# ArsamAryandoust/CarParkingMaps

Measured on AMD Instinct MI355X. Metric: car-steps/sec at Z=4,096, 1k cars/zone; 1/2/4/8 MI355X + %HBM roofline, higher is better.
Workload: dtype f64

## Files before the change

### carparkingmaps_amd/csrc/cpm_grouped.h

```cpp
#pragma once
#include <hip/hip_runtime.h>
#include <stdint.h>

#include <algorithm>
#include <cstring>
#include <type_traits>
#include <string>

#include "../../include/cpm.h"
#include "cpm_kernels.h"
#include "cpm_dispatch.h"
#include "cpm_narrow.h"
#include "cpm_flows.h"
#include "cpm_flows_csr.h"
#include "cpm_stays.h"
#include "cpm_paths.h"
#include "cpm_charge.h"

namespace cpm {

constexpr int kFusedThreads = 256;
constexpr int kMaxZonesPerGroup = 1024;
constexpr uint32_t kHiMax = 0xFFFFFFFFu;
constexpr int kMaxCapMult = 64;
// ... 153 lines not shown
    int Z, Zq, G;
    int hour;
    uint32_t *done_t;
    int lag;
    uint32_t heavy_x;
    uint32_t spin_limit;
    const uint32_t *pD, *pcntg;
    int pchunks;
    uint32_t cap, scap, idbits, gdiv, step;
    CarIndex cars;
    uint64_t seed;
    int Zc;
    int smap;
    uint32_t *sdone;
    const uint32_t *psdone;
    uint32_t *pdone;
    uint32_t chained;
    const uint32_t *perm_t;
};


__device__ __forceinline__ void lds_barrier() { asm volatile("s_waitcnt lgkmcnt(0)\n\ts_barrier" ::: "memory"); }

__device__ __forceinline__ unsigned long long ballot64(bool p) { return __builtin_amdgcn_ballot_w64(p); }
__device__ __forceinline__ uint32_t xcc_id() { return __builtin_amdgcn_s_getreg((20) | (0 << 6) | (3 << 11)) & 15u; }
__device__ __forceinline__ uint32_t wave_incl_scan(uint32_t x)
{
    int v = static_cast<int>(x);
    v += __builtin_amdgcn_update_dpp(0, v, 0x111, 0xf, 0xf, false);
    v += __builtin_amdgcn_update_dpp(0, v, 0x112, 0xf, 0xf, false);
    v += __builtin_amdgcn_update_dpp(0, v, 0x114, 0xf, 0xf, false);
    v += __builtin_amdgcn_update_dpp(0, v, 0x118, 0xf, 0xf, false);
    v += __builtin_amdgcn_update_dpp(0, v, 0x142, 0xa, 0xf, false);
    v += __builtin_amdgcn_update_dpp(0, v, 0x143, 0xc, 0xf, false);
    return static_cast<uint32_t>(v);
}
__device__ __forceinline__ bool any64(bool p) { return __builtin_amdgcn_ballot_w64(p) != 0ull; }
template <int POLICY, typename W>
__device__ __forceinline__ void next_store(W v, W *p);
template <int POLICY = 0>
__device__ __forceinline__ void put32(uint32_t *p, uint32_t i, uint32_t v)
{
    next_store<POLICY>(v, reinterpret_cast<uint32_t *>(reinterpret_cast<char *>(p) + (i << 2)));
}
__device__ __forceinline__ uint32_t from_lane0(uint32_t v) { return static_cast<uint32_t>(__builtin_amdgcn_readfirstlane(static_cast<int>(v))); }

constexpr int kRowTile = 64;
constexpr int kRowBlock = 256;
constexpr int kCkptStride = 32;
__host__ __device__ inline int ckpt_count(int Z) { return (Z + kCkptStride - 1) / kCkptStride; }
constexpr size_t kRowLds = sizeof(double) * 2 * kRowTile * (kRowTile + 1) + sizeof(uint32_t) * kRowTile;

typedef uint32_t cpm_u32x2 __attribute__((ext_vector_type(2)));
typedef uint32_t cpm_u32x4 __attribute__((ext_vector_type(4)));
__device__ __forceinline__ double row_load(__amdgpu_buffer_rsrc_t rows, uint32_t lane_off, uint32_t row_off)
{
    const cpm_u32x2 v = __builtin_amdgcn_raw_buffer_load_b64(rows, lane_off, row_off, 0);
    return __hiloint2double(static_cast<int>(v.y), static_cast<int>(v.x));
}

__device__ __forceinline__ void row_sums(double (*tile)[kRowTile][kRowTile + 1], const double *__restrict__ src, int lane, bool live,
                                         double *__restrict__ ck, double *__restrict__ last_o, int Z, int nt, int *err)
{
    constexpr int H = kRowTile / 2;
    const uint32_t lane_off = static_cast<uint32_t>(live ? lane : 0) << 3;
    const size_t Zs = static_cast<size_t>(Z);
    const uint32_t rowb = static_cast<uint32_t>(Z) * 8u;
    double run = 0.0;
    bool bad = false;
    double xa[H], xb[H];
    auto window = [&](const double *row0) {
        return __builtin_amdgcn_make_buffer_rsrc(const_cast<double *>(row0), 0, static_cast<int>(2 * kRowTile * rowb), 0x00020000);
    };
    auto sums = [&](double(&x)[H], int buf, int jbase, double *ck_slot) {
#pragma unroll
        for (int u = 0; u < H; ++u) {
            bad |= !(x[u] >= 0.0);
            run = run + x[u];
            tile[buf][lane][jbase + u] = run;
        }
        if (ck_slot && live) *ck_slot = run;
    };
    const int nfull = Z / kRowTile;
    const double *row0 = src;
    __amdgpu_buffer_rsrc_t rows = window(row0);
    if (nfull > 0) {
#pragma unroll
        for (int u = 0; u < H; ++u) xa[u] = row_load(rows, lane_off, static_cast<uint32_t>(u) * rowb);
    }
#pragma unroll 1
    for (int k = 0; k + 1 < nfull; ++k) {
#pragma unroll
        for (int u = 0; u < H; ++u) xb[u] = row_load(rows, lane_off, static_cast<uint32_t>(H + u) * rowb);
        sums(xa, k & 1, 0, ck ? ck + static_cast<size_t>(2 * k) * Zs : nullptr);
#pragma unroll
        for (int u = 0; u < H; ++u) xa[u] = row_load(rows, lane_off, static_cast<uint32_t>(kRowTile + u) * rowb);
        sums(xb, k & 1, H, ck ? ck + static_cast<size_t>(2 * k + 1) * Zs : nullptr);
        lds_barrier();
        row0 += kRowTile * Zs;
        rows = window(row0);
    }
    if (nfull > 0) {
        const int k = nfull - 1;
#pragma unroll
        for (int u = 0; u < H; ++u) xb[u] = row_load(rows, lane_off, static_cast<uint32_t>(H + u) * rowb);
        sums(xa, k & 1, 0, ck ? ck + static_cast<size_t>(2 * k) * Zs : nullptr);
// ... 456 lines not shown
__host__ __device__ constexpr int policy_sorted(int p) { return (p >> 2) & 3; }
__host__ __device__ constexpr int policy_medium(int p) { return (p >> 4) & 3; }
__host__ __device__ constexpr int policy_surplus(int p) { return (p >> 6) & 3; }
__host__ __device__ constexpr int policy_pack_aux(int p) { return ((p >> 8) & 1) ? 2 : 0; }
#ifndef CPM_HOUR_STAY
#define CPM_HOUR_STAY 0
#endif
#ifndef CPM_HOUR_SORTED
#define CPM_HOUR_SORTED 0
#endif
#ifndef CPM_HOUR_MEDIUM
#define CPM_HOUR_MEDIUM 0
#endif
#ifndef CPM_HOUR_SURPLUS
#define CPM_HOUR_SURPLUS 0
#endif
#ifndef CPM_HOUR_PACK_NT
#define CPM_HOUR_PACK_NT 1
#endif
#ifndef CPM_PAIR_STAY
#define CPM_PAIR_STAY 0
#endif
#ifndef CPM_PAIR_SORTED
#define CPM_PAIR_SORTED 0
#endif
#ifndef CPM_PAIR_SURPLUS
#define CPM_PAIR_SURPLUS 0
#endif
#ifndef CPM_PAIR_PACK_NT
#define CPM_PAIR_PACK_NT 1
#endif
#ifndef CPM_ZERO_STORE
#define CPM_ZERO_STORE 0
#endif
__host__ __device__ constexpr int policy_dense_pack_only(int p, bool sparse) { return sparse ? (p & 0xFF) : p; }
constexpr int kPolicyHour = store_policy(CPM_HOUR_STAY, CPM_HOUR_SORTED, CPM_HOUR_MEDIUM, CPM_HOUR_SURPLUS, CPM_HOUR_PACK_NT);
constexpr int kPolicyPair = store_policy(CPM_PAIR_STAY, CPM_PAIR_SORTED, 0, CPM_PAIR_SURPLUS, CPM_PAIR_PACK_NT);
template <bool FUSED>
__device__ __forceinline__ uint32_t hand_load(const uint32_t *p)
{
    if constexpr (FUSED) return __hip_atomic_load(p, __ATOMIC_RELAXED, __HIP_MEMORY_SCOPE_AGENT);
    else return *p;
}
template <bool FUSED>
__device__ __forceinline__ void hand_off_done(uint32_t *done_chunk, int tid)
{
    if constexpr (FUSED) {
        asm volatile("s_waitcnt vmcnt(0)" ::: "memory");
        __builtin_amdgcn_s_barrier();
        if (tid == 0) __hip_atomic_fetch_add(done_chunk, 1u, __ATOMIC_RELAXED, __HIP_MEMORY_SCOPE_AGENT);
    }
}

template <int BLOCK, int CPT, int NQ, bool GROUPED, bool FUSED, bool WAIT = false, bool SPARSE = false, bool STAGED = false, int POLICY = 0, bool NARROW = false>
__device__ __forceinline__ void grouped_sample_body(const GroupedArgs &a, const int z, uint32_t *pack, SampleLds &sl, uint32_t *done_chunk,
                                                    const uint32_t *wait_on = nullptr, uint32_t wait_need = 0)
{
    static_assert(!(STAGED && (WAIT || FUSED)), "a staged pack is the batched sampler's: two launches per hour");
    static_assert(!NARROW || (FUSED && GROUPED && !WAIT && !SPARSE && !STAGED), "narrow packs: the one-launch hour on dense tables");
    uint32_t &s_ndrive = sl.ndrive, &s_nstay = sl.nstay, &s_split = sl.split;
    uint32_t(&gb)[kGroups] = sl.gb;
    uint32_t(&stage)[kGroups * kStage] = sl.stage;
    const int tid = threadIdx.x, lane = tid & 63;
    const uint32_t cap = a.cap;
    const uint32_t b = static_cast<uint32_t>(z) * cap;
    const int gw = pack_guide_words(a.G), rw = NARROW ? narrow_row_words(a.Zq, a.G) : pack_row_words(a.Zq, a.G, SPARSE ? 1 : 0), pieces = rw / 4, sh = 32 - a.G;
    CPM_SSTAMP_DECL;
    CPM_SSTAMP(0);
    uint32_t ns_raw = a.cnt_s[z];
    if constexpr (WAIT) ns_raw &= kCntMask;
    const double last = a.last_t[z];
    const long long thr = a.thr_t[z];
    uint32_t na_raw;
    uint32_t id[CPT + 1];
    if constexpr (WAIT) {
        typedef uint32_t u32x2 __attribute__((ext_vector_type(2)));
        u32x2 seen = {wait_need, 0u};
        const bool poller = wait_need && tid < 64;
        if (poller) asm volatile("global_load_dwordx2 %0, %1, %2 sc1" : "=v"(seen) : "v"(0), "s"(wait_on) : "memory");
        pack_dma<BLOCK, NQ>(pack, a.rp_t + static_cast<size_t>(z) * rw, pieces, tid);
        if (poller) {
            asm volatile("s_waitcnt vmcnt(%1)" : "+v"(seen) : "n"(NQ) : "memory");
            uint32_t got = from_lane0(seen.x), where = from_lane0(seen.y);
            for (uint32_t spins = 0; (got & kDoneCount) < wait_need; ++spins) {
                if (spins >= a.spin_limit) break;
                __builtin_amdgcn_s_sleep(32);
                got = from_lane0(lane == 0 ? __hip_atomic_load(wait_on, __ATOMIC_RELAXED, __HIP_MEMORY_SCOPE_AGENT) : 0u);
                where = from_lane0(lane == 0 ? __hip_atomic_load(wait_on + 1, __ATOMIC_RELAXED, __HIP_MEMORY_SCOPE_AGENT) : 0u);
            }
            const bool bad = (got & kDoneCount) < wait_need || (got >> 16) != 0u || where != (1u << xcc_id());
            if (bad && lane == 0) atomicOr(a.rare->status, 4ull);
            if (tid == 0) sl.pad_ = bad ? 1u : 0u;
        }
        bool dead = false;
        if (wait_need) {
            lds_barrier();
            dead = sl.pad_ != 0u;
        }
        const uint32_t nsc = dead ? 0u : min(ns_raw, cap);
        uint32_t nav = 0;
        if (!dead) {
            asm volatile("global_load_dword %0, %1, %2 sc1" : "=v"(nav) : "v"(0), "s"(a.cnt_a + z) : "memory");
#pragma unroll
            for (int c = 0; c <= CPT; ++c) {
                const uint32_t s1 = static_cast<uint32_t>(tid + c * BLOCK);
                const uint32_t pos = s1 < nsc ? s1 : (cap - 1u + nsc - min(s1, cap - 1u + nsc));
                asm volatile("global_load_dword %0, %1, %2 sc1" : "=v"(id[c]) : "v"(pos << 2), "s"(a.ids + b) : "memory");
// ... 24 lines not shown
            asm volatile("global_load_dword %0, %1, %2" : "=v"(id[c]) : "v"(off), "s"(a.ids + b) : "memory");
        }
        if constexpr (STAGED) {
            wait_ids<CPT + 1, 0>(id);
        } else {
            pack_dma<BLOCK, NQ, policy_pack_aux(POLICY)>(pack, a.rp_t + static_cast<size_t>(z) * rw, pieces, tid);
            wait_ids<CPT + 1, NQ>(id);
        }
    }
    CPM_SSTAMP(1);
    const bool heavy = n_all > a.heavy_x * (CPT > 4 ? 4 : CPT) * BLOCK;
    if (tid == 0) {
        a.parking_t[z] = n_all;
        if (static_cast<unsigned long long>(ns_raw) + na_raw > cap) atomicOr(a.rare->status, 2ull);
        s_ndrive = 0;
        s_nstay = 0;
        uint32_t split = 0;
        if (heavy) {
            const GroupedRare *r = a.rare;
            const uint32_t items = (n_all + CPT * BLOCK - 1) / (CPT * BLOCK) - 1u;
            atomicMax(&r->maxn[0], n_all);
            const uint32_t idx = atomicAdd(r->nheavy + a.hour, items);
            atomicMax(&r->maxn[1], idx + items);
            if (GROUPED && r->parts > 1) {
                if (idx + items <= r->hgrid) {
                    for (uint32_t q = 0; q < items; ++q) r->heavy_list[idx + q] = static_cast<uint32_t>(z) | (q << 16);
                    split = 1;
                } else {
                    for (uint32_t q = 0; q < items && idx + q < r->hgrid; ++q) r->heavy_list[idx + q] = 0xFFFFFFFFu;
                }
            }
        }
        s_split = split;
    }
    if (tid < kGroups) gb[tid] = 0;
    if (n_all == 0) {
        if (GROUPED) {
            if (tid == 0) a.cnt_next[z] = 0;
            if (tid < kGroups) hand_store<FUSED>(&a.cntg[static_cast<size_t>(z) * kGroups + tid], 0u);
        }
        asm volatile("s_waitcnt vmcnt(0)" ::: "memory");
        hand_off_done<FUSED>(done_chunk, tid);
        return;
    }
    uint32_t nd = 0;
    uint32_t n = 0;
    const unsigned long long below = (1ull << lane) - 1ull;
    uint32_t *stay_out = a.ids_next + static_cast<size_t>(z) * cap;
    uint32_t *runs = GROUPED ? a.D + static_cast<size_t>(z) * kGroups * a.scap : nullptr;
    const uint16_t *guide = reinterpret_cast<const uint16_t *>(pack);
    const uint32_t *hi = pack + gw;
    const uint16_t *smap = SPARSE ? reinterpret_cast<const uint16_t *>(hi + a.Zq) : nullptr;
    uint32_t hi_last = 0;
    auto first_pass = [&](auto kc) {
        constexpr int K = decltype(kc)::value;
        bool valid[K ? K : 1], drive[K ? K : 1], want[K ? K : 1], ok[K ? K : 1];
        uint32_t dest[K ? K : 1], clo[K ? K : 1], khi[K ? K : 1];
#pragma unroll
        for (int c = 0; c < K; ++c) {
            valid[c] = static_cast<uint32_t>(tid + c * BLOCK) < n_all;
            long long kb;
            car_draw_words(a.seed, a.cars.global(id[c]), a.step, kb, clo[c], khi[c]);
            drive[c] = valid[c] & (kb <= thr);
            want[c] = drive[c] & (last != 0.0);
        }
        CPM_SSTAMP(2);
        asm volatile("s_waitcnt vmcnt(0)" ::: "memory");
        __syncthreads();
        CPM_SSTAMP(3);
        n = s_split ? static_cast<uint32_t>(CPT * BLOCK) : n_all;
        if constexpr (NARROW) hi_last = hi[0];
        else hi_last = hi[(SPARSE ? a.Zc : a.Z) - 1];
        if constexpr (K > 0) {
            if constexpr (NARROW) narrow_pack_search<K>(pack, gw, khi, want, sh, hi_last, a.Z, a.Zq, a.rare, a.hour, z, dest, ok);
            else pack_search<K>(guide, hi, khi, want, sh, hi_last, a.Zq, dest, ok, smap);
            {
                bool anyx = false;
#pragma unroll
                for (int c = 0; c < K; ++c) {
                    dest[c] = want[c] ? dest[c] : static_cast<uint32_t>(z);
                    anyx |= want[c] & !ok[c];
                }
                if (__builtin_expect(any64(anyx), 0)) {
#pragma unroll
                    for (int c = 0; c < K; ++c) {
                        if (want[c] & !ok[c]) {
                            if constexpr (NARROW) {
                                long long kb;
                                car_draw_words(a.seed, a.cars.global(id[c]), a.step, kb, clo[c], khi[c]);
                            }
                            dest[c] = search_exact_any<SPARSE>(a.rare, a.hour, z, u53(clo[c], khi[c]), last, khi[c] <= hi_last ? static_cast<int>(dest[c]) : -1);
                        }
                    }
                }
            }
            CPM_SSTAMP(4);
            if (GROUPED) {
                unsigned long long mS[K];
                uint32_t total = 0;
#pragma unroll
                for (int c = 0; c < K; ++c) {
                    mS[c] = ballot64(valid[c] & !drive[c]);
                    total += static_cast<uint32_t>(__popcll(mS[c]));
                }
                uint32_t bS = 0;
                if (lane == 0 && total) bS = atomicAdd(&s_nstay, total);
                bS = from_lane0(bS);
                uint32_t rank[K];
#pragma unroll
                for (int c = 0; c < K; ++c) rank[c] = drive[c] ? atomicAdd(&gb[gdiv_group_t<SPARSE>(a.gdiv, dest[c])], 1u) : 0u;
#pragma unroll
                for (int c = 0; c < K; ++c) {
                    if (valid[c] & !drive[c]) put32<policy_stay(POLICY)>(stay_out, bS + static_cast<uint32_t>(__popcll(mS[c] & below)), id[c]);
                    bS += static_cast<uint32_t>(__popcll(mS[c]));
                }
#pragma unroll
                for (int c = 0; c < K; ++c) {
                    if (drive[c]) {
                        const uint32_t g = gdiv_group_t<SPARSE>(a.gdiv, dest[c]);
                        const uint32_t packed = id[c] | (gdiv_local_t<SPARSE>(a.gdiv, dest[c], g) << a.idbits);
                        if (rank[c] < static_cast<uint32_t>(kStage)) stage[g * kStage + rank[c]] = packed;
                        else if (rank[c] < a.scap) hand_store<FUSED>(&runs[g * a.scap + rank[c]], packed);
                    }
                }
            } else {
#pragma unroll
// ... 16 lines not shown
            case 4: first_pass(std::integral_constant<int, 4>{}); break;
            case 5: first_pass(std::integral_constant<int, 5>{}); break;
            case 6: first_pass(std::integral_constant<int, 6>{}); break;
            case 7: first_pass(std::integral_constant<int, 7>{}); break;
            default: first_pass(std::integral_constant<int, 8>{}); break;
            }
        } else if constexpr (CPT == 7) {
            switch (k) {
            case 0: first_pass(std::integral_constant<int, 0>{}); break;
            case 1: first_pass(std::integral_constant<int, 1>{}); break;
            case 2: first_pass(std::integral_constant<int, 2>{}); break;
            case 3: first_pass(std::integral_constant<int, 3>{}); break;
            case 4: first_pass(std::integral_constant<int, 4>{}); break;
            case 5: first_pass(std::integral_constant<int, 5>{}); break;
            case 6: first_pass(std::integral_constant<int, 6>{}); break;
            default: first_pass(std::integral_constant<int, 7>{}); break;
            }
        } else if constexpr (CPT == 6) {
            switch (k) {
            case 0: first_pass(std::integral_constant<int, 0>{}); break;
            case 1: first_pass(std::integral_constant<int, 1>{}); break;
            case 2: first_pass(std::integral_constant<int, 2>{}); break;
            case 3: first_pass(std::integral_constant<int, 3>{}); break;
            case 4: first_pass(std::integral_constant<int, 4>{}); break;
            case 5: first_pass(std::integral_constant<int, 5>{}); break;
            default: first_pass(std::integral_constant<int, 6>{}); break;
            }
        } else if constexpr (CPT == 5) {
            switch (k) {
            case 0: first_pass(std::integral_constant<int, 0>{}); break;
            case 1: first_pass(std::integral_constant<int, 1>{}); break;
            case 2: first_pass(std::integral_constant<int, 2>{}); break;
            case 3: first_pass(std::integral_constant<int, 3>{}); break;
            case 4: first_pass(std::integral_constant<int, 4>{}); break;
            default: first_pass(std::integral_constant<int, 5>{}); break;
            }
        } else if constexpr (CPT == 4) {
            switch (k) {
            case 0: first_pass(std::integral_constant<int, 0>{}); break;
            case 1: first_pass(std::integral_constant<int, 1>{}); break;
            case 2: first_pass(std::integral_constant<int, 2>{}); break;
            case 3: first_pass(std::integral_constant<int, 3>{}); break;
            default: first_pass(std::integral_constant<int, 4>{}); break;
            }
        } else if constexpr (CPT == 2) {
            switch (k) {
            case 0: first_pass(std::integral_constant<int, 0>{}); break;
            case 1: first_pass(std::integral_constant<int, 1>{}); break;
            default: first_pass(std::integral_constant<int, 2>{}); break;
            }
        } else {
            if (k == 0) first_pass(std::integral_constant<int, 0>{});
            else first_pass(std::integral_constant<int, 1>{});
        }
    }
    for (uint32_t q0 = CPT * BLOCK; q0 < n; q0 += BLOCK) {
        if (q0 + static_cast<uint32_t>(tid & ~63) >= n) continue;
        const uint32_t q = q0 + tid;
        const bool valid1 = q < n;
        uint32_t idx;
        if constexpr (WAIT) idx = (q0 == CPT * BLOCK) ? id[CPT] : (valid1 ? hand_load<true>(&a.ids[b + (q < ns ? q : cap - 1u + ns - q)]) : 0u);
        else idx = (q0 == CPT * BLOCK) ? id[CPT] : (valid1 ? a.ids[b + q + (q >= ns ? cap - n_all : 0u)] : 0u);
        const uint64_t car = a.cars.global(idx);
        long long kb;
        uint32_t clo1[1], khi1[1], dest1[1];
        bool ok1[1], want1[1];
        car_draw_words(a.seed, car, a.step, kb, clo1[0], khi1[0]);
        const bool drive1 = valid1 & (kb <= thr);
        want1[0] = drive1 & (last != 0.0);
        if constexpr (NARROW) narrow_pack_search<1>(pack, gw, khi1, want1, sh, hi_last, a.Z, a.Zq, a.rare, a.hour, z, dest1, ok1);
        else pack_search<1>(guide, hi, khi1, want1, sh, hi_last, a.Zq, dest1, ok1, smap);
        if (!want1[0]) dest1[0] = z;
        else if (!ok1[0]) dest1[0] = search_exact_any<SPARSE>(a.rare, a.hour, z, u53(clo1[0], khi1[0]), last, khi1[0] <= hi_last ? static_cast<int>(dest1[0]) : -1);
        if (GROUPED) {
            const unsigned long long m1 = ballot64(valid1 & !drive1);
            uint32_t b1 = 0;
            if (lane == 0 && m1) b1 = atomicAdd(&s_nstay, static_cast<uint32_t>(__popcll(m1)));
            b1 = from_lane0(b1);
            if (valid1 & !drive1) next_store<policy_stay(POLICY)>(idx, &stay_out[b1 + static_cast<uint32_t>(__popcll(m1 & below))]);
            if (drive1) {
                const uint32_t g = gdiv_group_t<SPARSE>(a.gdiv, dest1[0]);
                const uint32_t rank = atomicAdd(&gb[g], 1u);
                const uint32_t packed = idx | (gdiv_local_t<SPARSE>(a.gdiv, dest1[0], g) << a.idbits);
                if (rank < static_cast<uint32_t>(kStage)) stage[g * kStage + rank] = packed;
                else if (rank < a.scap) hand_store<FUSED>(&runs[g * a.scap + rank], packed);
            }
        } else {
            if (valid1) stay_out[q] = dest1[0] | (drive1 ? kDriveBit : 0u);
            nd += drive1 ? 1u : 0u;
        }
    }
    if (!GROUPED) {
        for (int o = 32; o > 0; o >>= 1) nd += __shfl_down(nd, o, 64);
        if (lane == 0 && nd) atomicAdd(&s_ndrive, nd);
    }
    CPM_SSTAMP(5);
    lds_barrier();
    CPM_SSTAMP(6);
    if (GROUPED) {
        static_assert(kStage % 4 == 0, "16-byte pieces");
        const __amdgpu_buffer_rsrc_t rs = __builtin_amdgcn_make_buffer_rsrc(runs, 0, static_cast<int>(kGroups * a.scap * 4u), 0x00020000);
        for (int i = tid; i < kGroups * (kStage / 4); i += BLOCK) {
            const int g = i / (kStage / 4), ch = i % (kStage / 4);
            const uint32_t lim = min(gb[g], static_cast<uint32_t>(kStage));
            if (static_cast<uint32_t>(4 * ch) < lim) {
                const uint4 q = *reinterpret_cast<const uint4 *>(&stage[g * kStage + 4 * ch]);
// ... 475 lines not shown
    }
    static_assert(policy_surplus(POLICY) == place_surplus_policy<FUSED, SIGNAL, TAG>(), "the surplus helper and the body that calls it name the same policy");
    if (any_long) place_surplus_out<PB, KRUNS, KDEEP, ZPG, FUSED, SIGNAL, PERM, TAG>(pl, D, g, zs0, zs1, scap, idbits, zg0, nzl, cap, ids_next, ltotal);
    CPM_PSTAMP(7);
#if defined(CPM_DIAGNOSTIC) && !defined(CPM_STAMP_SAMPLER) && !defined(CPM_STAMP_BOTH)
    st_[7] = (st_[7] & ~1ull) | (any_long ? 1ull : 0ull);
#endif
#if defined(CPM_DIAGNOSTIC) && defined(CPM_STAMP_BOTH)
    st_[0] = (st_[0] & ~0xFFull) | ((__builtin_amdgcn_s_getreg((4) | (8 << 6) | (7 << 11))) & 0xFFu);
    st_[7] = (st_[7] & ~0x1Full) | xcc_id();
#endif
    CPM_PSTAMP_FLUSH;
    if constexpr (SIGNAL) {
        asm volatile("s_waitcnt vmcnt(0)" ::: "memory");
        __builtin_amdgcn_s_barrier();
        if (tid == 0) {
            __hip_atomic_fetch_or(done_out + 1, 1u << xcc_id(), __ATOMIC_RELAXED, __HIP_MEMORY_SCOPE_AGENT);
            __hip_atomic_fetch_add(done_out, 1u, __ATOMIC_RELAXED, __HIP_MEMORY_SCOPE_AGENT);
        }
    }
}

template <int PB, int KRUNS, int KDEEP>
__global__ __launch_bounds__(PB) void k_grouped_place(const uint32_t *__restrict__ D, const uint32_t *__restrict__ cntg, int zpg, int zps,
                                                               int Z, uint32_t cap, uint32_t scap, uint32_t idbits,
                                                               uint32_t *__restrict__ cnt_a_next, uint32_t *__restrict__ ids_next,
                                                               unsigned long long *status)
{
    __shared__ PlaceLds<PB, KRUNS, kMaxZonesPerGroup> pl;
    extern __shared__ uint32_t sorted_ids[];
    grouped_place_body<PB, KRUNS, KDEEP, kMaxZonesPerGroup, false, false, false, 0, kPolicyPair>(blockIdx.x % kGroups, blockIdx.x / kGroups, pl, sorted_ids, D, cntg, zpg, zps, Z, cap,
                                                                    scap, idbits, cnt_a_next, ids_next, status, nullptr, 0u, 0u);
}

#ifndef CPM_FUSED_KRUNS
#define CPM_FUSED_KRUNS 4
#endif
constexpr int kFusedKruns = CPM_FUSED_KRUNS;
#ifndef CPM_FUSED_KDEEP
#define CPM_FUSED_KDEEP 2
#endif
constexpr int kFusedKdeep = CPM_FUSED_KDEEP;
constexpr int kFusedChunk = 16 * kFusedKruns;
constexpr int kDoneStride = 32;

template <int CPT, int NQ, bool SPARSE, bool PERM, bool NARROW>
__device__ __forceinline__ void grouped_hour_block(const GroupedArgs &a)
{
    extern __shared__ uint32_t dyn[];
    __shared__ union {
        SampleLds s;
        PlaceLds<kFusedThreads, kFusedKruns, kFusedZpg> p;
    } u;
    constexpr int per = kFusedChunk + kGroups;
    const int nchunk = (a.Z + kFusedChunk - 1) / kFusedChunk;
    int z = -1, g = 0, j = -1;
    if (a.lag >= nchunk) {
        const int zr = (a.Z + 7) & ~7;
        if (static_cast<int>(blockIdx.x) < zr) {
            z = blockIdx.x;
            if (z >= a.Z) return;
            if constexpr (PERM) z = static_cast<int>(a.perm_t[blockIdx.x]);
        } else {
            const int b = blockIdx.x - zr;
            g = b % kGroups;
            j = b / kGroups;
        }
    } else {
        const int c = blockIdx.x / per, q = blockIdx.x % per;
        if (q < kFusedChunk) {
            z = c * kFusedChunk + q;
            if (c >= nchunk || z >= a.Z) return;
        } else {
            g = q - kFusedChunk;
            j = c - a.lag;
            if (j < 0) return;
        }
    }
    if (z >= 0) {
        grouped_sample_body<kFusedThreads, CPT, NARROW ? narrow_nq(NQ) : NQ, true, true, false, SPARSE, false, policy_dense_pack_only(kPolicyHour, SPARSE), NARROW>(
            a, z, dyn, u.s, a.done_t + static_cast<size_t>((PERM ? static_cast<int>(blockIdx.x) : z) / kFusedChunk) * kDoneStride);
    } else {
        const uint32_t need = static_cast<uint32_t>(min(kFusedChunk, a.Z - j * kFusedChunk));
#ifdef CPM_PLACE_PRIO
        __builtin_amdgcn_s_setprio(CPM_PLACE_PRIO);
#endif
        grouped_place_body<kFusedThreads, kFusedKruns, kFusedKdeep, kFusedZpg, true, false, PERM, 0, kPolicyHour>(
            g, j, u.p, dyn, a.D, a.cntg, static_cast<int>(gdiv_zpg(a.gdiv)), kFusedChunk, a.Z, a.cap, a.scap, a.idbits, a.cnt_next + a.Z, a.ids_next, a.rare->status,
            a.done_t + static_cast<size_t>(j) * kDoneStride, need, a.spin_limit, nullptr, PERM ? a.perm_t : nullptr, SPARSE);
    }
}
template <int CPT, int NQ, bool SPARSE = false, bool PERM = false>
__global__ __launch_bounds__(kFusedThreads, CPM_WPS) CPM_SGPR_ATTR void k_grouped_hour(GroupedArgs a)
{
    grouped_hour_block<CPT, NQ, SPARSE, PERM, false>(a);
}
template <int CPT, int NQ>
__global__ __launch_bounds__(kFusedThreads, CPM_WPS) CPM_SGPR_ATTR void k_grouped_hour_narrow(GroupedArgs a)
{
    grouped_hour_block<CPT, NQ, false, false, true>(a);
}

template <int CPT, int NQ, bool GROUPED, bool SPARSE = false>
__global__ __launch_bounds__(kFusedThreads, CPM_WPS) CPM_SGPR_ATTR void k_grouped_hour_pf(GroupedArgs a)
{
    extern __shared__ uint32_t dyn[];
    __shared__ union {
        SampleLds s;
        PlaceLds<kFusedThreads, kFusedKruns, kFusedZpg> p;
    } u;
    const int npl = a.pchunks * kGroups;
    if (static_cast<int>(blockIdx.x) < npl) {
        const int b = blockIdx.x;
        const int g = (b / (8 * a.pchunks)) * 8 + (b & 7), j = (b >> 3) % a.pchunks;
        grouped_place_body<kFusedThreads, kFusedKruns, kFusedKdeep, kFusedZpg, false, true>(
            g, j, u.p, dyn, a.pD, a.pcntg, static_cast<int>(gdiv_zpg(a.gdiv)), kFusedChunk, a.Z, a.cap, a.scap, a.idbits, const_cast<uint32_t *>(a.cnt_a),
            const_cast<uint32_t *>(a.ids), a.rare->status, nullptr, 0u, 0u, a.done_t + static_cast<size_t>(g) * kDoneStride);
    } else {
        const int bs = blockIdx.x - npl, zpg = static_cast<int>(gdiv_zpg(a.gdiv));
        const int g = (bs & 7) + 8 * ((bs >> 3) / zpg), z = g * zpg + ((bs >> 3) % zpg);
        if (g >= kGroups || z >= a.Z) return;
        grouped_sample_body<kFusedThreads, CPT, NQ, GROUPED, false, true, SPARSE>(a, z, dyn, u.s, nullptr, a.done_t + static_cast<size_t>(g) * kDoneStride,
                                                                          static_cast<uint32_t>(a.pchunks));
    }
}

struct LaunchCells {
    uint32_t applied = 0, heavy = 0, last = 0, place = 0, batch = 0;
    bool hour_T = false;
    bool narrow = false;
    void sampler(uint32_t word) { (hour_T ? last : applied) = word; }
};
inline LaunchCells &launch_cells()
// ... 296 lines not shown
            double2 cell = make_double2(0.0, 0.0);
            if (moving) cell = tt_row[dest[u]];
            mean[u] = cell.x;
            sd[u] = cell.y;
        }
#pragma unroll
        for (int u = 0; u < kTravelBatch; ++u) {
            if (!live[u]) continue;
            if (dest[u] == static_cast<uint32_t>(z)) {
                tt += q16(300.0);
            } else {
                const double s1 = (sd[u] == 0) ? 0.1 * mean[u] : sd[u];
                tt += q16(truncnormal_pm10(tr.seed, tr.cars.global(w[u] & idmask), step, 1, mean[u], s1));
            }
        }
    }
    }
    for (int o = 32; o > 0; o >>= 1) tt += __shfl_down(tt, o, 64);
    if (lane == 0 && tt) atomicAdd(&s_tt, static_cast<unsigned long long>(tt));
    __syncthreads();
    if (tid == 0 && s_tt) atomicAdd(&tr.tt_part[(z + 31 * blockIdx.y) % kTravelParts], s_tt);
}

__global__ __launch_bounds__(256) void k_grouped_travel_finish(unsigned long long *__restrict__ tt_part, unsigned long long *__restrict__ tt_sum)
{
    unsigned long long v = tt_part[threadIdx.x];
    tt_part[threadIdx.x] = 0;
    for (int o = 32; o > 0; o >>= 1) v += __shfl_down(v, o, 64);
    if ((threadIdx.x & 63) == 0 && v) atomicAdd(tt_sum, v);
}

template <bool GROUPED, int CPT, int NQ, bool SPARSE>
inline hipError_t grouped_launch_sample_t(const GroupedArgs &a, size_t lds, hipStream_t stream)
{
    constexpr auto kernel = k_grouped_sample<kSampleBlock, CPT, NQ, GROUPED, SPARSE>;
    const hipError_t e = lds_opt_in<kernel>(lds, kPackLds);
    if (e != hipSuccess) return e;
    launch_cells().sampler(cell_word(kCellSample, CPT, NQ, GROUPED, SPARSE));
    launch(kernel, dim3(a.Z), dim3(kSampleBlock), lds, stream, a);
    return hipSuccess;
}
template <bool GROUPED>
inline hipError_t grouped_launch_sample(const GroupedArgs &a, int64_t mean, bool heavy_follows, hipStream_t stream)
{
    const size_t lds = sizeof(uint32_t) * static_cast<size_t>(pack_row_words(a.Zq, a.G, a.smap));
    return cell_walk<SampleCells>(heavy_follows ? grouped_cpt(mean) : grouped_cpt_wide(mean), pack_need(a.Zq, a.G, a.smap), a.smap != 0,
                                  [&](auto CPT, auto NQ, auto SPARSE) { return grouped_launch_sample_t<GROUPED, CPT, NQ, SPARSE>(a, lds, stream); });
}

inline size_t fused_lds_bytes(int Zq, int G, int smap = 0)
{
    return std::max(sizeof(uint32_t) * static_cast<size_t>(pack_row_words(Zq, G, smap)), static_cast<size_t>(4 + sizeof(PlaceLds<kFusedThreads, kFusedKruns, kFusedZpg>::zone_t)) * kFusedKruns * kFusedKdeep * kFusedThreads);
}
inline size_t fused_lds_bytes_narrow(int Zq, int G)
{
    return std::max(sizeof(uint32_t) * static_cast<size_t>(narrow_row_words(Zq, G)), fused_lds_bytes(0, 3));
}
template <int CPT, int NQ, bool SPARSE, bool PERM = false>
inline hipError_t grouped_launch_hour_t(const GroupedArgs &a, hipStream_t stream)
{
    const int nchunk = (a.Z + kFusedChunk - 1) / kFusedChunk;
    if constexpr (!PERM) {
        if (a.perm_t && a.lag >= nchunk)
            return grouped_launch_hour_t<CPT, NQ, SPARSE, true>(a, stream);
    }
    constexpr auto kernel = k_grouped_hour<CPT, NQ, SPARSE, PERM>;
    const size_t lds = fused_lds_bytes(a.Zq, a.G, a.smap);
    const hipError_t e = lds_opt_in<kernel>(lds, kPackLds);
    if (e != hipSuccess) return e;
    const unsigned blocks = a.lag >= nchunk ? static_cast<unsigned>(((a.Z + 7) & ~7) + nchunk * kGroups)
                                            : static_cast<unsigned>((nchunk + a.lag) * (kFusedChunk + kGroups));
    launch_cells().sampler(cell_word(kCellHour, CPT, NQ, true, SPARSE, PERM));
    launch(kernel, dim3(blocks), dim3(kFusedThreads), lds, stream, a);
    return hipSuccess;
}
inline bool fused_pays(int Z, int Zq, int G, int cu_count, int smap = 0, int64_t mean = 0)
{
    if (smap) return mean >= 256 && Z >= 6 * std::max(cu_count, 1);
    const size_t lds = fused_lds_bytes(Zq, G, smap) + 4608;
    return Z >= 12 * std::max(cu_count, 1) && 5 * lds <= 160 * 1024;
}
template <int CPT, int NQ>
inline hipError_t grouped_launch_hour_narrow_t(const GroupedArgs &a, hipStream_t stream)
{
    static_assert(sizeof(uint32_t) * 1024 * narrow_nq(NQ) <= kPackLds, "the narrow pack of every Z of the rung fits");
    const int nchunk = (a.Z + kFusedChunk - 1) / kFusedChunk;
    constexpr auto kernel = k_grouped_hour_narrow<CPT, NQ>;
    const size_t lds = fused_lds_bytes_narrow(a.Zq, a.G);
    if (narrow_need(a.Zq, a.G) > narrow_nq(NQ)) return hipErrorInvalidValue;
    const hipError_t e = lds_opt_in<kernel>(lds, kPackLds);
    if (e != hipSuccess) return e;
    const unsigned blocks = a.lag >= nchunk ? static_cast<unsigned>(((a.Z + 7) & ~7) + nchunk * kGroups)
                                            : static_cast<unsigned>((nchunk + a.lag) * (kFusedChunk + kGroups));
    launch_cells().sampler(cell_word(kCellHour, CPT, NQ, true, false, false));
    launch_cells().narrow = true;
    launch(kernel, dim3(blocks), dim3(kFusedThreads), lds, stream, a);
    return hipSuccess;
}
inline hipError_t grouped_launch_hour(const GroupedArgs &a, int64_t mean, hipStream_t stream, bool narrow = false)
{
    return cell_walk<HourCells>(grouped_cpt_wide(mean), pack_need(a.Zq, a.G, a.smap), a.smap != 0, [&](auto CPT, auto NQ, auto SPARSE) {
        if constexpr (!SPARSE) {
            if (narrow) return grouped_launch_hour_narrow_t<CPT, NQ>(a, stream);
        }
        return grouped_launch_hour_t<CPT, NQ, SPARSE>(a, stream);
    });
}

__global__ __launch_bounds__(256) void k_narrow_rows(const uint32_t *__restrict__ wide, uint32_t *__restrict__ narrow, int Z, int Zq, int G)
{
    struct WideRow {
        const uint32_t *w;
        __device__ NarrowPiece piece(int i) const
        {
            const uint4 v = reinterpret_cast<const uint4 *>(w)[i];
            return NarrowPiece{{v.x, v.y, v.z, v.w}};
        }
        __device__ uint32_t word(int i) const { return w[i]; }
    };
    const int rw = pack_row_words(Zq, G), rn = narrow_row_words(Zq, G);
    const WideRow row{wide + static_cast<size_t>(blockIdx.x) * rw};
    uint4 *o = reinterpret_cast<uint4 *>(narrow + static_cast<size_t>(blockIdx.x) * rn);
    for (int q = threadIdx.x; q < rn / 4; q += 256) {
        const NarrowPiece p = narrow_piece(row, q, Z, Zq, G);
        o[q] = make_uint4(p.v[0], p.v[1], p.v[2], p.v[3]);
    }
}
inline hipError_t narrow_build_rows(const uint32_t *wide, uint32_t *narrow, int64_t rows, int Z, int Zq, int G, hipStream_t stream)
{
    hipLaunchKernelGGL(k_narrow_rows, dim3(static_cast<unsigned>(rows)), dim3(256), 0, stream, wide, narrow, Z, Zq, G);
    return hipGetLastError();
}

template <int CPT, int NQ, bool GROUPED, bool SPARSE>
inline hipError_t grouped_launch_hour_pf_t(const GroupedArgs &a, hipStream_t stream)
{
    constexpr auto kernel = k_grouped_hour_pf<CPT, NQ, GROUPED, SPARSE>;
    const size_t lds = fused_lds_bytes(a.Zq, a.G, a.smap);
    const hipError_t e = lds_opt_in<kernel>(lds, kPackLds);
    if (e != hipSuccess) return e;
    launch_cells().sampler(cell_word(kCellHourPf, CPT, NQ, GROUPED, SPARSE));
// ... 625 lines not shown
```

### carparkingmaps_amd/csrc/cpm_narrow.h

```cpp
#pragma once
#include "cpm_dispatch.h"

#if defined(__HIPCC__)
#define CPM_UNROLL _Pragma("unroll")
#else
#define CPM_UNROLL
#endif
#if defined(__HIP_DEVICE_COMPILE__)
#define CPM_OPAQUE(x) asm volatile("" : "+v"(x))
#else
#define CPM_OPAQUE(x) (void)(x)
#endif

namespace cpm {

constexpr int kNarrowHeadWords = 4;

CPM_HD constexpr int narrow_shift(int G) { return 32 - G - 16; }
CPM_HD constexpr int narrow_row_words(int Zq, int G)
{
    const int w = pack_guide_words(G) + kNarrowHeadWords + Zq / 2;
    return w < 256 ? 256 : w;
}
constexpr int narrow_need(int Zq, int G) { return (narrow_row_words(Zq, G) / 4 + kSampleBlock - 1) / kSampleBlock; }
// ... 57 lines not shown
    }
    CPM_UNROLL
    for (int c = 0; c < CPT; ++c) {
        n[c] = in[c] ? n[c] - lo[c] : 0u;
        nor |= n[c];
    }
    uint32_t p[CPT], end[CPT];
    CPM_UNROLL
    for (int c = 0; c < CPT; ++c) {
        p[c] = a.cur(lo[c]);
        end[c] = p[c] + n[c] * kS;
    }
#define CPM_NARROW_STEP(S, AT)                                                                          \
    do {                                                                                                \
        uint32_t v_[CPT];                                                                               \
        CPM_UNROLL for (int c = 0; c < CPT; ++c) v_[c] = a.at(AT(p[c] + ((S) - 1u) * kS));              \
        CPM_UNROLL for (int c = 0; c < CPT; ++c) {                                                      \
            const uint32_t t_ = p[c] + (S) * kS;                                                        \
            p[c] = ((v_[c] < k16[c]) & (t_ <= end[c])) ? t_ : p[c];                                     \
        }                                                                                               \
    } while (0)
#define CPM_NARROW_AT_PAD(q) (q)
#define CPM_NARROW_AT_ROW(q) ((q) < top ? (q) : top)
    if (a.any(nor >= 32u)) {
        const uint32_t top = a.cur(static_cast<uint32_t>(Zq - 1));
        int K = 6;
        while (a.any((nor >> K) != 0u)) ++K;
        for (uint32_t s = 1u << (K - 1); s != 0u; s >>= 1) CPM_NARROW_STEP(s, CPM_NARROW_AT_ROW);
    } else {
        const bool a16 = a.any(nor >= 16u);
        const bool a8 = a16 || a.any(nor >= 8u);
        if (a16) CPM_NARROW_STEP(16u, CPM_NARROW_AT_PAD);
        if (a8) CPM_NARROW_STEP(8u, CPM_NARROW_AT_PAD);
        CPM_NARROW_STEP(4u, CPM_NARROW_AT_PAD);
        CPM_NARROW_STEP(2u, CPM_NARROW_AT_PAD);
        CPM_NARROW_STEP(1u, CPM_NARROW_AT_PAD);
    }
#undef CPM_NARROW_AT_ROW
#undef CPM_NARROW_AT_PAD
#undef CPM_NARROW_STEP
    CPM_UNROLL
    for (int c = 0; c < CPT; ++c) {
        const bool full = p[c] == end[c];
        const uint32_t fin = a.at(p[c]);
        dest[c] = a.idx(p[c]);
        uint32_t kq = khi[c];
        CPM_OPAQUE(kq);
        const bool inc = want[c] & (kq <= hi_last);
        tie[c] = inc & !full & (fin == k16[c]);
        ok[c] = inc & (full ? (dest[c] != static_cast<uint32_t>(Z - 1) || hi_last > khi[c]) : (fin > k16[c]));
    }
}

constexpr uint32_t kNarrowTieOk = 0x80000000u;
template <typename W>
CPM_HD inline uint32_t narrow_tie_walk(const W &w, uint32_t dest, uint32_t khi, int Z, int Zq)
{
    for (uint32_t j0 = dest; j0 < static_cast<uint32_t>(Zq); j0 += 4u) {
        uint32_t v[4];
        for (uint32_t i = 0; i < 4u; ++i) v[i] = w(j0 + i < static_cast<uint32_t>(Zq) ? j0 + i : static_cast<uint32_t>(Zq) - 1u);
        for (uint32_t i = 0; i < 4u; ++i)
            if (v[i] >= khi) return (j0 + i < static_cast<uint32_t>(Z) ? j0 + i : static_cast<uint32_t>(Z) - 1u) | (v[i] > khi ? kNarrowTieOk : 0u);
    }
    return static_cast<uint32_t>(Z) - 1u;
}

}
```

Before: 136.5 billion.

## Compact driving cars per wavefront into LDS before narrow pack search

In the fused narrow hour kernel, each wavefront ballots its driving cars and writes their id and key into a per-wave LDS scratch. It then runs the narrow pack search over densely packed slots, sized to the driving count rounded up to 64, rather than over every car slot. Stay cars are written out directly in the first pass. This removes divergent search work on lanes whose cars do not drive, at the cost of extra LDS scratch, which could lower occupancy, and more template instantiations. It is gated by a compile-time check that the extra LDS does not lower blocks per CU and by a CPT mask that disables it for CPT=2.

```diff
diff --git a/carparkingmaps_amd/csrc/cpm_grouped.h b/carparkingmaps_amd/csrc/cpm_grouped.h
--- a/carparkingmaps_amd/csrc/cpm_grouped.h
+++ b/carparkingmaps_amd/csrc/cpm_grouped.h
@@ -229,6 +229,7 @@
 constexpr size_t kRowLds = sizeof(double) * 2 * kRowTile * (kRowTile + 1) + sizeof(uint32_t) * kRowTile;
 
 typedef uint32_t cpm_u32x2 __attribute__((ext_vector_type(2)));
+typedef __attribute__((address_space(3))) cpm_u32x2 lds_u32x2;
 typedef uint32_t cpm_u32x4 __attribute__((ext_vector_type(4)));
 __device__ __forceinline__ double row_load(__amdgpu_buffer_rsrc_t rows, uint32_t lane_off, uint32_t row_off)
 {
@@ -791,7 +792,7 @@
     }
 }
 
-template <int BLOCK, int CPT, int NQ, bool GROUPED, bool FUSED, bool WAIT = false, bool SPARSE = false, bool STAGED = false, int POLICY = 0, bool NARROW = false>
+template <int BLOCK, int CPT, int NQ, bool GROUPED, bool FUSED, bool WAIT = false, bool SPARSE = false, bool STAGED = false, int POLICY = 0, bool NARROW = false, bool DENSE_ON = false>
 __device__ __forceinline__ void grouped_sample_body(const GroupedArgs &a, const int z, uint32_t *pack, SampleLds &sl, uint32_t *done_chunk,
                                                     const uint32_t *wait_on = nullptr, uint32_t wait_need = 0)
 {
@@ -922,6 +923,10 @@
     const uint32_t *hi = pack + gw;
     const uint16_t *smap = SPARSE ? reinterpret_cast<const uint16_t *>(hi + a.Zq) : nullptr;
     uint32_t hi_last = 0;
+    constexpr bool DENSE = NARROW && GROUPED && DENSE_ON;
+    uint32_t ndrv = 0;
+    lds_u32x2 *scr = nullptr;
+    if constexpr (DENSE) scr = (lds_u32x2 *)(pack + rw) + static_cast<uint32_t>(tid >> 6) * dense_cap(CPT);
     auto first_pass = [&](auto kc) {
         constexpr int K = decltype(kc)::value;
         bool valid[K ? K : 1], drive[K ? K : 1], want[K ? K : 1], ok[K ? K : 1];
@@ -933,6 +938,20 @@
             car_draw_words(a.seed, a.cars.global(id[c]), a.step, kb, clo[c], khi[c]);
             drive[c] = valid[c] & (kb <= thr);
             want[c] = drive[c] & (last != 0.0);
+        }
+        if constexpr (DENSE && K > 0) {
+#pragma unroll
+            for (int c = 0; c < K; ++c) {
+                const unsigned long long m = ballot64(drive[c]);
+                const uint32_t rk = dense_rank(m, lane, ndrv);
+                if (drive[c]) {
+                    cpm_u32x2 v;
+                    v.x = id[c];
+                    v.y = khi[c];
+                    scr[rk] = v;
+                }
+                ndrv += static_cast<uint32_t>(__popcll(m));
+            }
         }
         CPM_SSTAMP(2);
         asm volatile("s_waitcnt vmcnt(0)" ::: "memory");
@@ -941,7 +960,25 @@
         n = s_split ? static_cast<uint32_t>(CPT * BLOCK) : n_all;
         if constexpr (NARROW) hi_last = hi[0];
         else hi_last = hi[(SPARSE ? a.Zc : a.Z) - 1];
-        if constexpr (K > 0) {
+        if constexpr (DENSE) {
+            if constexpr (K > 0) {
+                unsigned long long mS[K];
+                uint32_t total = 0;
+#pragma unroll
+                for (int c = 0; c < K; ++c) {
+                    mS[c] = ballot64(valid[c] & !drive[c]);
+                    total += static_cast<uint32_t>(__popcll(mS[c]));
+                }
+                uint32_t bS = 0;
+                if (lane == 0 && total) bS = atomicAdd(&s_nstay, total);
+                bS = from_lane0(bS);
+#pragma unroll
+                for (int c = 0; c < K; ++c) {
+                    if (valid[c] & !drive[c]) put32<policy_stay(POLICY)>(stay_out, bS + static_cast<uint32_t>(__popcll(mS[c] & below)), id[c]);
+                    bS += static_cast<uint32_t>(__popcll(mS[c]));
+                }
+            }
+        } else if constexpr (K > 0) {
             if constexpr (NARROW) narrow_pack_search<K>(pack, gw, khi, want, sh, hi_last, a.Z, a.Zq, a.rare, a.hour, z, dest, ok);
             else pack_search<K>(guide, hi, khi, want, sh, hi_last, a.Zq, dest, ok, smap);
             {
@@ -1064,6 +1101,63 @@
         } else {
             if (k == 0) first_pass(std::integral_constant<int, 0>{});
             else first_pass(std::integral_constant<int, 1>{});
+        }
+    }
+    if constexpr (DENSE) {
+        auto dense_pass = [&](auto kdc) {
+            constexpr int KD = decltype(kdc)::value;
+            uint32_t did[KD], dkhi[KD], ddest[KD], rank[KD];
+            bool live[KD], dwant[KD], dok[KD];
+#pragma unroll
+            for (int s = 0; s < KD; ++s) {
+                const cpm_u32x2 v = scr[dense_read_pos(s, lane)];
+                did[s] = v.x;
+                dkhi[s] = v.y;
+                live[s] = dense_live(s, KD, lane, ndrv);
+                dwant[s] = live[s] & (last != 0.0);
+            }
+            narrow_pack_search<KD>(pack, gw, dkhi, dwant, sh, hi_last, a.Z, a.Zq, a.rare, a.hour, z, ddest, dok);
+            bool anyx = false;
+#pragma unroll
+            for (int s = 0; s < KD; ++s) {
+                ddest[s] = dwant[s] ? ddest[s] : static_cast<uint32_t>(z);
+                anyx |= dwant[s] & !dok[s];
+            }
+            if (__builtin_expect(any64(anyx), 0)) {
+#pragma unroll
+                for (int s = 0; s < KD; ++s) {
+                    if (dwant[s] & !dok[s]) {
+                        long long kb;
+                        uint32_t lo_w, hi_w;
+                        car_draw_words(a.seed, a.cars.global(did[s]), a.step, kb, lo_w, hi_w);
+                        ddest[s] = search_exact_any<SPARSE>(a.rare, a.hour, z, u53(lo_w, hi_w), last, hi_w <= hi_last ? static_cast<int>(ddest[s]) : -1);
+                    }
+                }
+            }
+            CPM_SSTAMP(4);
+#pragma unroll
+            for (int s = 0; s < KD; ++s) rank[s] = live[s] ? atomicAdd(&gb[gdiv_group_t<SPARSE>(a.gdiv, ddest[s])], 1u) : 0u;
+#pragma unroll
+            for (int s = 0; s < KD; ++s) {
+                if (live[s]) {
+                    const uint32_t g = gdiv_group_t<SPARSE>(a.gdiv, ddest[s]);
+                    const uint32_t packed = did[s] | (gdiv_local_t<SPARSE>(a.gdiv, ddest[s], g) << a.idbits);
+                    if (rank[s] < static_cast<uint32_t>(kStage)) stage[g * kStage + rank[s]] = packed;
+                    else if (rank[s] < a.scap) hand_store<FUSED>(&runs[g * a.scap + rank[s]], packed);
+                }
+            }
+        };
+        static_assert(CPT <= 8, "the dispatch below");
+        switch (dense_round_slots(ndrv)) {
+        case 0: break;
+        case 1: dense_pass(std::integral_constant<int, 1>{}); break;
+        case 2: dense_pass(std::integral_constant<int, CPT >= 2 ? 2 : CPT>{}); break;
+        case 3: dense_pass(std::integral_constant<int, CPT >= 3 ? 3 : CPT>{}); break;
+        case 4: dense_pass(std::integral_constant<int, CPT >= 4 ? 4 : CPT>{}); break;
+        case 5: dense_pass(std::integral_constant<int, CPT >= 5 ? 5 : CPT>{}); break;
+        case 6: dense_pass(std::integral_constant<int, CPT >= 6 ? 6 : CPT>{}); break;
+        case 7: dense_pass(std::integral_constant<int, CPT >= 7 ? 7 : CPT>{}); break;
+        default: dense_pass(std::integral_constant<int, CPT>{}); break;
         }
     }
     for (uint32_t q0 = CPT * BLOCK; q0 < n; q0 += BLOCK) {
@@ -1645,6 +1739,7 @@
         SampleLds s;
         PlaceLds<kFusedThreads, kFusedKruns, kFusedZpg> p;
     } u;
+    static_assert(sizeof(u) == kFusedStaticLds && kFusedThreads == kDenseBlock, "dense_fits (cpm_narrow.h) counts these bytes");
     constexpr int per = kFusedChunk + kGroups;
     const int nchunk = (a.Z + kFusedChunk - 1) / kFusedChunk;
     int z = -1, g = 0, j = -1;
@@ -1671,7 +1766,7 @@
         }
     }
     if (z >= 0) {
-        grouped_sample_body<kFusedThreads, CPT, NARROW ? narrow_nq(NQ) : NQ, true, true, false, SPARSE, false, policy_dense_pack_only(kPolicyHour, SPARSE), NARROW>(
+        grouped_sample_body<kFusedThreads, CPT, NARROW ? narrow_nq(NQ) : NQ, true, true, false, SPARSE, false, policy_dense_pack_only(kPolicyHour, SPARSE), NARROW, NARROW && dense_on(CPT, NQ)>(
             a, z, dyn, u.s, a.done_t + static_cast<size_t>((PERM ? static_cast<int>(blockIdx.x) : z) / kFusedChunk) * kDoneStride);
     } else {
         const uint32_t need = static_cast<uint32_t>(min(kFusedChunk, a.Z - j * kFusedChunk));
@@ -2074,9 +2169,11 @@
 {
     return std::max(sizeof(uint32_t) * static_cast<size_t>(pack_row_words(Zq, G, smap)), static_cast<size_t>(4 + sizeof(PlaceLds<kFusedThreads, kFusedKruns, kFusedZpg>::zone_t)) * kFusedKruns * kFusedKdeep * kFusedThreads);
 }
-inline size_t fused_lds_bytes_narrow(int Zq, int G)
-{
-    return std::max(sizeof(uint32_t) * static_cast<size_t>(narrow_row_words(Zq, G)), fused_lds_bytes(0, 3));
+static_assert((4 + sizeof(PlaceLds<kFusedThreads, kFusedKruns, kFusedZpg>::zone_t)) * kFusedKruns * kFusedKdeep * kFusedThreads == kFusedListLds,
+              "dense_fits (cpm_narrow.h) counts the placing list's bytes: CPM_FUSED_LIST_LDS");
+inline size_t fused_lds_bytes_narrow(int Zq, int G, int cpt, int rung)
+{
+    return std::max(sizeof(uint32_t) * static_cast<size_t>(narrow_row_words(Zq, G)) + dense_scratch_bytes(kFusedThreads, cpt, rung), fused_lds_bytes(0, 3));
 }
 template <int CPT, int NQ, bool SPARSE, bool PERM = false>
 inline hipError_t grouped_launch_hour_t(const GroupedArgs &a, hipStream_t stream)
@@ -2108,7 +2205,7 @@
     static_assert(sizeof(uint32_t) * 1024 * narrow_nq(NQ) <= kPackLds, "the narrow pack of every Z of the rung fits");
     const int nchunk = (a.Z + kFusedChunk - 1) / kFusedChunk;
     constexpr auto kernel = k_grouped_hour_narrow<CPT, NQ>;
-    const size_t lds = fused_lds_bytes_narrow(a.Zq, a.G);
+    const size_t lds = fused_lds_bytes_narrow(a.Zq, a.G, CPT, NQ);
     if (narrow_need(a.Zq, a.G) > narrow_nq(NQ)) return hipErrorInvalidValue;
     const hipError_t e = lds_opt_in<kernel>(lds, kPackLds);
     if (e != hipSuccess) return e;
diff --git a/carparkingmaps_amd/csrc/cpm_narrow.h b/carparkingmaps_amd/csrc/cpm_narrow.h
--- a/carparkingmaps_amd/csrc/cpm_narrow.h
+++ b/carparkingmaps_amd/csrc/cpm_narrow.h
@@ -133,6 +133,48 @@
     }
 }
 
+constexpr uint32_t kDensePayloadBytes = 8;
+CPM_HD constexpr uint32_t dense_cap(int cpt) { return 64u * static_cast<uint32_t>(cpt); }
+#ifndef CPM_DENSE_CPT_MASK
+#define CPM_DENSE_CPT_MASK (~(1u << 2))
+#endif
+CPM_HD constexpr bool dense_pays(int cpt) { return ((static_cast<uint32_t>(CPM_DENSE_CPT_MASK) >> cpt) & 1u) != 0u; }
+constexpr size_t kCuLdsBytes = 160 * 1024, kLdsStep = 1280;
+constexpr size_t kFusedStaticLds = 4240;
+#ifndef CPM_FUSED_LIST_LDS
+#define CPM_FUSED_LIST_LDS 10240
+#endif
+constexpr size_t kFusedListLds = CPM_FUSED_LIST_LDS;
+constexpr int kDenseBlock = 256;
+constexpr int dense_blocks_by_registers(int cpt) { return cpt >= 6 ? 6 : 7; }
+constexpr size_t dense_scratch_raw(int block, int cpt) { return static_cast<size_t>(block / 64) * dense_cap(cpt) * kDensePayloadBytes; }
+constexpr size_t lds_step_up(size_t b) { return (b + kLdsStep - 1) / kLdsStep * kLdsStep; }
+constexpr bool dense_fits(int cpt, int rung)
+{
+    const int top = narrow_band_top(rung);
+    const size_t pack = sizeof(uint32_t) * static_cast<size_t>(narrow_row_words(pack_zq(top), pack_guide_bits(top)));
+    const size_t before = (pack > kFusedListLds ? pack : kFusedListLds) + kFusedStaticLds;
+    const size_t scr = pack + dense_scratch_raw(kDenseBlock, cpt);
+    const size_t after = lds_step_up((scr > kFusedListLds ? scr : kFusedListLds) + kFusedStaticLds);
+    const size_t by_lds = kCuLdsBytes / before, by_reg = static_cast<size_t>(dense_blocks_by_registers(cpt));
+    return after * (by_lds < by_reg ? by_lds : by_reg) <= kCuLdsBytes;
+}
+constexpr bool dense_on(int cpt, int rung) { return dense_pays(cpt) && dense_fits(cpt, rung); }
+static_assert(dense_fits(6, 5) && !dense_fits(6, 6) && dense_fits(4, 5) && !dense_fits(4, 6), "the headline compacts; six / seven blocks per CU are kept above Z = 4,096");
+constexpr size_t dense_scratch_bytes(int block, int cpt, int rung) { return dense_on(cpt, rung) ? dense_scratch_raw(block, cpt) : 0; }
+CPM_HD inline uint32_t dense_rank(unsigned long long m, int lane, uint32_t before)
+{
+#if defined(__HIP_DEVICE_COMPILE__)
+    (void)lane;
+    return __builtin_amdgcn_mbcnt_hi(static_cast<uint32_t>(m >> 32), __builtin_amdgcn_mbcnt_lo(static_cast<uint32_t>(m), before));
+#else
+    return before + static_cast<uint32_t>(__builtin_popcountll(m & ((1ull << lane) - 1ull)));
+#endif
+}
+CPM_HD constexpr uint32_t dense_round_slots(uint32_t count) { return (count + 63u) >> 6; }
+CPM_HD constexpr uint32_t dense_read_pos(int s, int lane) { return static_cast<uint32_t>(s) * 64u + static_cast<uint32_t>(lane); }
+CPM_HD constexpr bool dense_live(int s, int kd, int lane, uint32_t count) { return s < kd - 1 || dense_read_pos(s, lane) < count; }
+
 constexpr uint32_t kNarrowTieOk = 0x80000000u;
 template <typename W>
 CPM_HD inline uint32_t narrow_tie_walk(const W &w, uint32_t dest, uint32_t khi, int Z, int Zq)
```

Result: faster. 140.5 billion, median of 6 (+2.9%).
